# eth-cscs/COSTA

Hardware: AMD Instinct MI355X
Metric: GB/s device-resident tile pack+transpose+unpack (fp64), % HBM peak (higher is better)
Workload: dtype f64; 1 GPU; pxtran fp64 16384x16384, 256x256 blocks, op T, alpha=1 beta=0, 1x1 grid (BASELINE configs[1]); op=T, parallelism=1 rank(s), one per GPU, RCCL send/recv exchange, m=16384, n=16384, block=256, grid=1x1

## Files before the change

costa_amd/__init__.py:

```python
from __future__ import annotations

import ctypes as C
import os
import struct
from dataclasses import dataclass
from typing import Iterable, Sequence

import numpy as np

__all__ = [
    "CostaError", "lib", "FLOAT", "DOUBLE", "CFLOAT", "CDOUBLE", "INT32", "HALF", "BFLOAT16",
    "FP8_E4M3", "FP8_E5M2", "dtype_code", "element_code",
    "np_dtype", "Layout", "block_cyclic_layout", "custom_layout", "Comm", "transform",
    "transform_batch", "transform_async", "transform_batch_async", "synchronize", "transformer", "copy_and_transform", "execute_tiles", "execute_tiles_mixed",
    "convert_subtile", "TileOp", "TriOp", "TRI_OP_DTYPE", "transform_tri", "transform_tri_async",
    "execute_tiles_tri", "plan_export_tri", "tri_cut", "tri_subtile", "tri_phase_ms",
    "plan_export", "set_profiling", "get_stats", "release_caches", "TILE_OP_DTYPE",
    "ScaledOp", "SCALED_OP_DTYPE", "SCALED_F_ROWS", "transform_scaled", "execute_tiles_scaled",
    "plan_export_scaled", "scaled_subtile", "scaled_items",
    "transform_amax", "layout_amax", "execute_tiles_amax", "amax_items",
]

FLOAT, DOUBLE, CFLOAT, CDOUBLE, INT32 = 0, 1, 2, 3, 4
HALF, BFLOAT16 = 5, 6
# ... 179 lines not shown
        "costa_hip_transform_tri": (i, [vp, vp, c, c, i, vp, vp, vp]),
        "costa_hip_transform_tri_async": (i, [vp, vp, c, c, i, vp, vp, vp, vp]),
        "costa_hip_execute_tiles_tri": (i, [i, C.POINTER(TriOp), i64, vp, vp, vp, i, i]),
        "costa_hip_tri_cut": (i, []),
        "costa_hip_tri_phase_ms": (i, [C.POINTER(C.c_double), i]),
        "costa_hip_tri_subtile": (i, [i, C.POINTER(i), C.POINTER(i)]),
        "costa_hip_plan_export_tri": (i, [vp, vp, c, c, i, vp, vp, i, i, C.POINTER(TriPlanInfo), vp, vp,
                                          vp, vp, vp, vp, vp, vp, vp, vp]),
        "costa_hip_transform_scaled": (i, [vp, vp, c, vp, vp, vp, vp, vp]),
        "costa_hip_transform_scaled_async": (i, [vp, vp, c, vp, vp, vp, vp, vp, vp]),
        "costa_hip_execute_tiles_scaled": (i, [i, i, C.POINTER(ScaledOp), i64, vp, vp, vp, i, vp, vp, i]),
        "costa_hip_scaled_subtile": (i, [i, i, C.POINTER(i), C.POINTER(i)]),
        "costa_hip_scaled_items": (i, [C.POINTER(i64), i]),
        "costa_hip_transform_amax": (i, [vp, vp, c, vp, vp, vp, vp, vp, vp, vp]),
        "costa_hip_transform_amax_async": (i, [vp, vp, c, vp, vp, vp, vp, vp, vp, vp, vp]),
        "costa_hip_layout_amax": (i, [vp, vp, vp, vp]),
        "costa_hip_layout_amax_async": (i, [vp, vp, vp, vp, vp]),
        "costa_hip_execute_tiles_amax": (i, [i, i, C.POINTER(ScaledOp), i64, vp, vp, vp, i, vp, vp, vp, vp,
                                             i]),
        "costa_hip_amax_items": (i, [C.POINTER(i64), i]),
        "costa_hip_plan_export_scaled": (i, [vp, vp, c, vp, vp, i, i, C.POINTER(ScaledPlanInfo), vp, vp,
                                             vp, vp, vp, vp, vp, vp]),
        "costa_hip_plan_export": (i, [i, C.POINTER(vp), C.POINTER(vp), C.c_char_p, vp, vp, i, i,
                                      C.POINTER(PlanInfo), vp, vp, vp, vp, vp, vp, vp, vp]),
        "costa_hip_set_profiling": (i, [i]),
        "costa_hip_get_stats": (i, [C.POINTER(FullStats), i]),
        "costa_hip_release_caches": (i, []),
        "costa_hip_set_host_staging": (i, [i]),
        "costa_hip_set_planner": (i, [i]),
        "costa_hip_plan_export_device": (i, [i, i, C.POINTER(vp), C.POINTER(vp), C.c_char_p, vp, vp,
                                             i, i, C.POINTER(PlanInfo), vp, vp, vp, vp, vp, vp, vp,
                                             vp]),
        "costa_hip_set_list_builder": (i, [i]),
        "costa_hip_work_export": (i, [i, vp, i64, i, i, vp, i64, vp, i64, C.POINTER(i64)]),
    }
    for name, (res, args) in sig.items():
        try:
            f = getattr(L, name)
        except AttributeError:
            if os.environ.get("COSTA_LIB"):
                continue
            raise
        f.restype = res
        f.argtypes = args
    _lib = L
    return L


def _check(rc: int):
    if rc != 0:
        raise CostaError(rc, lib().costa_hip_last_error().decode(errors="replace"))


def _ptr(p) -> int:
    if p is None:
        return 0
    if isinstance(p, int):
        return p
    if isinstance(p, np.ndarray):
        return p.ctypes.data
    if hasattr(p, "data_ptr"):
        return p.data_ptr()
    raise TypeError(f"cannot take the address of {type(p)}")


def _scalar_bytes(code: int, x) -> bytes:
# ... 16 lines not shown
    row_start: int
    row_end: int
    col_start: int
    col_end: int
    data: int
    ld: int


class Layout:

    def __init__(self, handle: int, dtype: int, keep: Iterable = ()):
        self._h = C.c_void_p(handle)
        self.dtype = dtype
        self._keep = list(keep)

    @property
    def handle(self) -> C.c_void_p:
        return self._h

    def num_blocks(self) -> int:
        return lib().costa_hip_layout_num_blocks(self._h)

    def block(self, i: int) -> BlockInfo:
        v = [C.c_int() for _ in range(4)]
        d, ld = C.c_void_p(), C.c_int()
        _check(lib().costa_hip_layout_block(self._h, i, *[C.byref(x) for x in v], C.byref(d),
                                            C.byref(ld)))
        return BlockInfo(v[0].value, v[1].value, v[2].value, v[3].value, d.value or 0, ld.value)

    def shape(self) -> tuple:
        m, n = C.c_int(), C.c_int()
        _check(lib().costa_hip_layout_shape(self._h, C.byref(m), C.byref(n)))
        return m.value, n.value

    def reorder_ranks(self, reordering: Sequence[int]):
        p = np.ascontiguousarray(reordering, dtype=np.int32)
        _check(lib().costa_hip_layout_reorder_ranks(self._h, p.ctypes.data_as(C.POINTER(C.c_int)),
                                                    int(p.size)))

    def close(self):
        if self._h and self._h.value:
            lib().costa_hip_layout_destroy(self._h)
            self._h = C.c_void_p(0)

    def __del__(self):
        try:
            self.close()
        except Exception:
            pass


def block_cyclic_layout(m, n, block_m, block_n, i, j, sub_m, sub_n, p_m, p_n, order, rsrc, csrc,
                        ptr, lld, ordering, rank, dtype=DOUBLE) -> Layout:
    code = element_code(dtype)
    h = C.c_void_p()
    _check(lib().costa_hip_block_cyclic_layout(code, m, n, block_m, block_n, i, j, sub_m, sub_n,
                                               p_m, p_n, _chr(order), rsrc, csrc,
                                               C.c_void_p(_ptr(ptr)), lld, _chr(ordering), rank,
                                               C.byref(h)))
    return Layout(h.value, code, [ptr])


def custom_layout(rowblocks, colblocks, rowsplit, colsplit, owners, localblocks, ordering,
                  dtype=DOUBLE) -> Layout:
    code = element_code(dtype)
    rs = np.ascontiguousarray(rowsplit, dtype=np.int32)
# ... 459 lines not shown
    L = lib()
    args = (A.handle, Cl.handle, _chr(trans), ab, bb, rank, nranks, C.byref(info))
    _check(L.costa_hip_plan_export_scaled(*args, *([None] * 8)))
    b = info.base
    po = np.zeros(b.n_pack, TILE_OP_DTYPE)
    ls = np.zeros(info.n_local_scaled, SCALED_OP_DTYPE)
    us = np.zeros(info.n_unpack_scaled, SCALED_OP_DTYPE)
    cnt = [np.zeros(nranks, np.int64) for _ in range(4)]
    sc = np.zeros(2 * b.n_slots, _NP[code])
    _check(L.costa_hip_plan_export_scaled(*args, po.ctypes.data, ls.ctypes.data, us.ctypes.data,
                                          *[x.ctypes.data for x in cnt], sc.ctypes.data))
    return ScaledPlan(np.zeros(b.n_local, TILE_OP_DTYPE), po, np.zeros(b.n_unpack, TILE_OP_DTYPE), *cnt,
                      sc, b.send_elems, b.recv_elems, b.local_elems, ls, us)


def set_profiling(on: bool = True):
    _check(lib().costa_hip_set_profiling(int(on)))


def get_stats(reset: bool = False) -> dict:
    s = FullStats()
    _check(lib().costa_hip_get_stats(C.byref(s), int(reset)))
    return s.as_dict()


def release_caches():
    _check(lib().costa_hip_release_caches())


def set_planner(mode: int):
    _check(lib().costa_hip_set_planner(int(mode)))


def set_list_builder(mode: int):
    _check(lib().costa_hip_set_list_builder(int(mode)))


@dataclass
class WorkLists:
    ordered: np.ndarray
    work: np.ndarray
    meta: dict
    on_gpu: bool


_WORK_META = ("n_large", "n_medium", "n_skew", "n_cblock", "cblock_lds", "cb_map", "tiny_first",
              "n_tiny", "n_ordered", "n_work", "on_gpu", "flags")


def work_export(dtype, ops: np.ndarray, kind: str = "local", device=None) -> WorkLists:
    code = element_code(dtype)
    ops = np.ascontiguousarray(ops, dtype=TILE_OP_DTYPE)
    k = {"local": 0, "pack": 1, "unpack": 2}[kind]
    dev = -1 if device is None else int(device)
    meta = (C.c_int64 * 12)()
    L = lib()
    _check(L.costa_hip_work_export(code, ops.ctypes.data, ops.size, k, dev, None, 0, None, 0, meta))
    o = np.zeros(meta[8], TILE_OP_DTYPE)
    w = np.zeros(meta[9], np.uint64)
    _check(L.costa_hip_work_export(code, ops.ctypes.data, ops.size, k, dev, o.ctypes.data, o.size,
                                   w.ctypes.data, w.size, meta))
    m = dict(zip(_WORK_META, list(meta)))
    return WorkLists(o, w, m, bool(m["on_gpu"]))


def set_host_staging(mode: int):
# ... 8 lines not shown
```

costa_amd/csrc/capi.cpp:

```cpp
#include "engine.hpp"

#include <hip/hip_runtime.h>

#include <costa/transform.hpp>

#include <algorithm>
#include <cctype>
#include <complex>
#include <cstring>
#include <new>

struct costa_layout_s {
    costa::engine::elayout e;
    std::vector<int> base_owners;
};
struct costa_comm_s {
    costa::engine::comm* c = nullptr;
};

namespace {
thread_local std::string g_last_error;

template <typename F>
int guarded(F&& f) {
// ... 674 lines not shown
        [&](const std::vector<job>& jobs) { return costa::engine::make_plan(jobs, rank, nranks); },
        n, A, C, trans, alpha, beta, rank, nranks, info, local_ops, pack_ops, unpack_ops,
        send_counts, send_displs, recv_counts, recv_displs, scalars);
}

int costa_hip_plan_export_device(int device, int n, const costa_layout_t* A, const costa_layout_t* C,
                                 const char* trans, const void* alpha, const void* beta, int rank,
                                 int nranks, costa_plan_info_t* info, costa_tile_op_t* local_ops,
                                 costa_tile_op_t* pack_ops, costa_tile_op_t* unpack_ops,
                                 int64_t* send_counts, int64_t* send_displs, int64_t* recv_counts,
                                 int64_t* recv_displs, void* scalars) {
    device_restore keep;
    return export_plan(
        [&](const std::vector<job>& jobs) {
            auto p = costa::engine::make_plan_device(jobs, rank, nranks, 0, device, nullptr);
            if (!p)
                throw costa::engine::error(COSTA_ERR_ARG,
                                           "costa: the device planner does not apply to these "
                                           "layouts (local blocks are not exactly the rank's grid "
                                           "cells)");
            return p;
        },
        n, A, C, trans, alpha, beta, rank, nranks, info, local_ops, pack_ops, unpack_ops,
        send_counts, send_displs, recv_counts, recv_displs, scalars);
}

int costa_hip_set_planner(int mode) {
    return guarded([&] {
        if (mode < 0 || mode > 2) throw costa::engine::error(COSTA_ERR_ARG, "mode must be 0, 1 or 2");
        costa::engine::set_planner_mode(mode);
    });
}

int costa_hip_set_list_builder(int mode) {
    return guarded([&] {
        if (mode < 0 || mode > 2) throw costa::engine::error(COSTA_ERR_ARG, "mode must be 0, 1 or 2");
        costa::engine::set_list_builder_mode(mode);
    });
}

int costa_hip_work_export(int dtype, const costa_tile_op_t* ops, int64_t n_ops, int kind, int device,
                          costa_tile_op_t* ordered, int64_t cap_ordered, uint64_t* work,
                          int64_t cap_work, int64_t* meta) {
    auto body = [&] {
        if (!meta || (n_ops > 0 && !ops) || n_ops < 0) throw costa::engine::error(COSTA_ERR_ARG, "null argument");
        if (dtype < COSTA_FLOAT || dtype > COSTA_INT32) throw costa::engine::error(COSTA_ERR_ARG, "bad dtype");
        if (kind < 0 || kind > 2) throw costa::engine::error(COSTA_ERR_ARG, "kind must be 0, 1 or 2");
        std::vector<costa_tile_op_t> in(ops, ops + n_ops), o;
        std::vector<uint64_t> w;
        costa::engine::work_split ws;
        const bool on_gpu = costa::engine::work_export(
            costa_dtype_t(dtype), in, costa::engine::list_kind(kind), device, o, w, ws);
        const int64_t m[12] = {ws.n_large, ws.n_medium, ws.n_skew, ws.n_cblock, ws.cblock_lds, ws.cb_map,
                               ws.tiny_first, ws.n_tiny, int64_t(o.size()), int64_t(w.size()), on_gpu,
                               int64_t(ws.tr_shape) | int64_t(ws.sq) << 1 | int64_t(ws.full) << 2 |
                                   int64_t(ws.med_full) << 3 | int64_t(ws.med_sq) << 4 |
                                   int64_t(ws.skew_wide) << 5};
        std::memcpy(meta, m, sizeof(m));
        if (ordered && cap_ordered >= int64_t(o.size()) && !o.empty())
            std::memcpy(ordered, o.data(), o.size() * sizeof(o[0]));
        if (work && cap_work >= int64_t(w.size()) && !w.empty()) std::memcpy(work, w.data(), w.size() * sizeof(w[0]));
    };
    return device >= 0 ? gpu_guarded(body) : guarded(body);
}

int costa_hip_set_profiling(int on) {
// ... 166 lines not shown
```

costa_amd/csrc/engine.cpp:

```cpp
#include <exception>
#include <thread>
#include "engine.hpp"
#include "strip_work.hpp"

#include <hip/hip_runtime.h>
#include <rccl/rccl.h>

#include <algorithm>
#include <numeric>
#include <chrono>
#include <cmath>
#include <cstdio>
#include <cstdlib>
#include <cstring>
#include <deque>
#include <list>
#include <map>
#include <mutex>
#include <unordered_map>

namespace costa {
namespace engine {

#define HIP_CHECK(x)                                                                   \
// ... 1442 lines not shown
namespace {
int g_host_mode = -1;
}
int host_staging_mode() {
    if (g_host_mode < 0) {
        const char* s = std::getenv("COSTA_HOST_STAGING");
        g_host_mode = s ? (std::atoi(s) != 0) : 1;
    }
    return g_host_mode;
}
void set_host_staging_mode(int mode) {
    std::lock_guard<std::recursive_mutex> lk(g_mutex);
    g_host_mode = mode != 0;
}

namespace {

struct hasher {
    uint64_t h = 0x9E3779B97F4A7C15ull;
    uint64_t h2 = 0x2545F4914F6CDD1Dull;
    void mix(uint64_t v) {
        v ^= v >> 33;
        v *= 0xff51afd7ed558ccdull;
        v ^= v >> 33;
        h = (h ^ v) * 0xc4ceb9fe1a85ec53ull + 0x165667b19e3779f9ull;
        h ^= h >> 29;
        h2 = (h2 + v) * 0x9fb21c651e98df25ull;
        h2 ^= h2 >> 31;
    }
    void mix_vec(const std::vector<int>& v) {
        mix(v.size());
        for (int x : v) mix(uint64_t(uint32_t(x)));
    }
    void mix_layout(const elayout& L) {
        mix(uint64_t(L.dtype));
        mix(uint64_t(uint8_t(L.ordering)));
        mix(uint64_t(L.n_ranks));
        mix_vec(L.rows_split);
        mix_vec(L.cols_split);
        mix_vec(L.owners);
        mix(L.blocks.size());
        for (const auto& b : L.blocks) {
            mix(uint64_t(uint32_t(b.rows.start)) | (uint64_t(uint32_t(b.rows.end)) << 32));
            mix(uint64_t(uint32_t(b.cols.start)) | (uint64_t(uint32_t(b.cols.end)) << 32));
            mix(reinterpret_cast<uintptr_t>(b.data));
            mix(uint64_t(uint32_t(b.ld)));
        }
    }
};

}

uint64_t layout_hash(const elayout& L) {
    hasher h;
    h.mix_layout(L);
    return h.h | 1;
}

void layout_hashes(const elayout& L, uint64_t& h1, uint64_t& h2) {
    hasher h;
    h.mix_layout(L);
    h1 = h.h | 1;
    h2 = h.h2;
}

void set_layout_hash(elayout& L) { layout_hashes(L, L.hash, L.hash2); }

namespace {

struct cached_plan {
    std::unique_ptr<plan> p;
    int device = 0;
    bool staged = false;
    std::vector<hrange> h2d_ranges, d2h_ranges;
    dbuf stage;
    dbuf d_local, w_local, d_scal;
    work_split l_local;
    bool tr_local = true, ax_local = true;
    strip_list c_local;
    dbuf d_local_tri, w_local_tri;
    strip_list t_local;
    dbuf d_local_sc, w_local_sc;
    strip_list s_local;
    struct xround {
        dbuf d_pack, w_pack, d_unpack, w_unpack;
        work_split l_pack, l_unpack;
        strip_list c_pack, c_unpack;
        dbuf d_unpack_tri, w_unpack_tri;
        strip_list t_unpack;
        dbuf d_unpack_sc, w_unpack_sc;
        strip_list s_unpack;
        bool tr_unpack = false, ax_unpack = false;
    };
    std::vector<std::unique_ptr<xround>> rounds;
    std::vector<unsigned char> scal_host;
    std::shared_ptr<host_pipeline> pipe;
};

constexpr size_t kMaxPlans = 16;
struct keyed_plan {
    uint64_t h = 0;
    std::vector<uint64_t> key;
    std::unique_ptr<cached_plan> plan;
};
std::list<keyed_plan> g_plans;

void key_layout(std::vector<uint64_t>& k, const elayout& L) {
    uint64_t h1 = L.hash, h2 = L.hash2;
    if (!h1) layout_hashes(L, h1, h2);
    k.push_back(h1);
    k.push_back(h2);
    k.push_back(uint64_t(L.dtype) | uint64_t(uint8_t(L.ordering)) << 8 |
                uint64_t(uint32_t(L.n_ranks)) << 32);
    k.push_back(uint64_t(uint32_t(L.nbr())) | uint64_t(uint32_t(L.nbc())) << 32);
    k.push_back(L.blocks.size());
    if (!L.blocks.empty())
        for (const eblock* b : {&L.blocks.front(), &L.blocks.back()}) {
            k.push_back(reinterpret_cast<uintptr_t>(b->data));
            k.push_back(uint64_t(uint32_t(b->ld)) | uint64_t(uint32_t(b->rows.start)) << 32);
        }
}

elayout remap(const elayout& L, const std::vector<hrange>& ranges, char* dev) {
    elayout out = L;
    for (auto& b : out.blocks) {
        uintptr_t p = reinterpret_cast<uintptr_t>(b.data);
        auto it = std::upper_bound(ranges.begin(), ranges.end(), p,
                                   [](uintptr_t v, const hrange& r) { return v < r.lo; });
        if (it == ranges.begin()) throw error(COSTA_ERR_INTERNAL, "costa: staging map miss");
        --it;
        b.data = dev + it->dev_off + (p - it->lo);
    }
    return out;
}

std::vector<hrange> collect_ranges(const std::vector<const elayout*>& Ls) {
    std::vector<hrange> r;
    for (const elayout* L : Ls) {
        const size_t E = dtype_size(L->dtype);
        for (const auto& b : L->blocks) {
            size_t ext = block_extent_bytes(b, L->ordering, E);
            if (!ext) continue;
            uintptr_t lo = reinterpret_cast<uintptr_t>(b.data);
            r.push_back({lo, lo + ext, 0});
        }
    }
    std::sort(r.begin(), r.end(), [](const hrange& x, const hrange& y) { return x.lo < y.lo; });
    std::vector<hrange> m;
    for (const auto& x : r) {
        if (!m.empty() && x.lo <= m.back().hi)
            m.back().hi = std::max(m.back().hi, x.hi);
        else
            m.push_back(x);
    }
    return m;
}

// ... 4 lines not shown
constexpr size_t kDevicePlanBlocks = 4096;
constexpr size_t kColdDevicePlanBlocks = 100000;
bool g_device_planner_warm = false;
}

int planner_mode() {
    if (g_planner < 0) {
        const char* s = std::getenv("COSTA_PLANNER");
        g_planner = s ? std::max(0, std::min(2, std::atoi(s))) : 1;
    }
    return g_planner;
}

void set_planner_mode(int mode) {
    std::lock_guard<std::recursive_mutex> lk(g_mutex);
    g_planner = mode;
}

namespace {
int g_list_builder = -1;
}

int list_builder_mode() {
    if (g_list_builder < 0) {
        const char* s = std::getenv("COSTA_LIST_BUILDER");
        g_list_builder = s ? std::max(0, std::min(2, std::atoi(s))) : 1;
    }
    return g_list_builder;
}

void set_list_builder_mode(int mode) {
    std::lock_guard<std::recursive_mutex> lk(g_mutex);
    g_list_builder = mode;
}

namespace {
template <typename X>
void upload_list(dbuf& d, const std::vector<X>& h, const X* sec, size_t at, size_t n, hipStream_t s) {
    if (!sec || n == 0) return d.upload(h, s);
    const size_t total = h.size() + n;
    d.reserve(total * sizeof(X));
    X* p = static_cast<X*>(d.p);
    if (at) HIP_CHECK(hipMemcpyAsync(p, h.data(), at * sizeof(X), hipMemcpyHostToDevice, s));
    HIP_CHECK(hipMemcpyAsync(p + at, sec, n * sizeof(X), hipMemcpyDeviceToDevice, s));
    if (h.size() > at)
        HIP_CHECK(hipMemcpyAsync(p + at + n, h.data() + at, (h.size() - at) * sizeof(X), hipMemcpyHostToDevice, s));
}
}

bool work_export(costa_dtype_t dtype, const std::vector<costa_tile_op_t>& ops, list_kind kind, int device,
                 std::vector<costa_tile_op_t>& ordered, std::vector<uint64_t>& work, work_split& w) {
    std::lock_guard<std::recursive_mutex> lk(g_mutex);
    if (device < 0) {
        w = build_work(dtype, ops, ordered, work, kind);
        return false;
    }
    device_ctx& dc = ctx(device);
    device_section sec;
    sec.device = device;
    sec.stream = dc.main;
    sec.force = true;
    w = build_work(dtype, ops, ordered, work, kind, &sec);
    if (!sec.n_ordered) return false;
    std::vector<costa_tile_op_t> o(sec.n_ordered);
    std::vector<uint64_t> k(sec.n_work);
    HIP_CHECK(hipMemcpyAsync(o.data(), sec.d_ordered, o.size() * sizeof(o[0]), hipMemcpyDeviceToHost, dc.main));
    HIP_CHECK(hipMemcpyAsync(k.data(), sec.d_work, k.size() * sizeof(k[0]), hipMemcpyDeviceToHost, dc.main));
    HIP_CHECK(hipStreamSynchronize(dc.main));
    ordered.insert(ordered.begin() + std::ptrdiff_t(sec.at_ordered), o.begin(), o.end());
    work.insert(work.begin() + std::ptrdiff_t(sec.at_work), k.begin(), k.end());
    return true;
}

namespace {
std::unique_ptr<plan> plan_jobs(const std::vector<job>& jobs, comm* c, hipStream_t s) {
    const int lb = c->size == 1 && c->nccl ? loopback_exchange() : 0;
    const int mode = planner_mode();
    size_t blocks = 0;
    for (const job& j : jobs) blocks += j.A->blocks.size() + j.C->blocks.size();
    const size_t need = g_device_planner_warm ? kDevicePlanBlocks : kColdDevicePlanBlocks;
    if (mode == 2 || (mode == 1 && blocks >= need)) {
        if (auto p = make_plan_device(jobs, c->rank, c->size, lb, c->device, s)) {
            g_stats.device_plans++;
            g_device_planner_warm = true;
            return p;
        }
    }
    return make_plan(jobs, c->rank, c->size, lb);
}

cached_plan* get_plan(const std::vector<job>& jobs, comm* c, device_ctx& dc) {
    std::vector<uint64_t> key;
    key.reserve(4 + jobs.size() * 30);
    key.push_back(uint64_t(uint32_t(c->rank)) | uint64_t(uint32_t(c->size)) << 32);
    key.push_back(uint64_t(uint32_t(c->device)) | uint64_t(uint32_t(host_staging_mode())) << 32);
    key.push_back(jobs.size());
    for (const auto& j : jobs) {
        key_layout(key, *j.A);
        key_layout(key, *j.C);
        uint64_t w = uint64_t(uint8_t(std::toupper(static_cast<unsigned char>(j.trans))));
        for (bool cm : {true, false})
            w = w << 8 | scale_kind(j.C->dtype, j.s, cm, std::toupper(j.trans) == 'C');
        key.push_back(w);
        key.push_back(uint64_t(uint8_t(std::toupper(static_cast<unsigned char>(j.uplo)))) << 32 |
                      uint64_t(j.scaled) << 40 | uint64_t(uint32_t(j.k)));
    }
    hasher h;
    for (uint64_t w : key) h.mix(w);
    for (auto it = g_plans.begin(); it != g_plans.end(); ++it) {
        if (it->h == h.h && it->key == key) {
            g_plans.splice(g_plans.begin(), g_plans, it);
            g_stats.plan_hits++;
            return g_plans.front().plan.get();
        }
    }
    g_stats.plan_misses++;
    static const bool trace = std::getenv("COSTA_PLAN_TRACE") != nullptr;
    auto now = [] {
        return std::chrono::duration<double, std::milli>(
                   std::chrono::steady_clock::now().time_since_epoch()).count();
    };
    const double t0 = now();
    double t_resid = 0, t_plan = 0, t_work = 0;

    const bool half = any_half(jobs);
    const bool fp8 = any_fp8(jobs);
    const bool mixed = any_mixed(jobs) || half || fp8;
    const bool masked = any_masked(jobs);
    const bool scaled = any_scaled(jobs);
    if (mixed || masked || scaled) {
        costa_dtype_t a, b;
        check_jobs(jobs, c->size, a, b);
    }
    auto cp = std::make_unique<cached_plan>();
    cp->device = c->device;
    bool all_dev = true;
    std::vector<const elayout*> host_layouts;
    std::vector<bool> on_dev;
    for (const auto& j : jobs)
        for (const elayout* L : {j.A, j.C}) {
            bool d = layout_on_device(*L);
            on_dev.push_back(d);
            all_dev = all_dev && d;
        }
    std::vector<elayout> remapped;
    std::vector<job> pj = jobs;
    std::vector<hrange> staged_ranges;
    std::vector<uint8_t> range_flags;
    if (!all_dev && mixed)
        throw error(COSTA_ERR_ARG,
                    fp8  ? "costa: FP8 transforms (A or C of a 1-byte element type) need "
                           "device-resident layouts"
                    : half ? "costa: half-precision transforms (A or C of a 2-byte element type) need "
                           "device-resident layouts"
                         : "costa: mixed-precision transforms (A and C of different element types) need "
                           "device-resident layouts");
    if (!all_dev && scaled)
        throw error(COSTA_ERR_ARG, "costa: scaled transforms need device-resident layouts");
    if (!all_dev) {
        cp->staged = true;
        std::vector<const elayout*> As, Cs;
        size_t k = 0;
        for (const auto& j : jobs) {
            if (!on_dev[k++]) As.push_back(j.A);
            if (!on_dev[k++]) Cs.push_back(j.C);
        }
        std::vector<const elayout*> all = As;
        all.insert(all.end(), Cs.begin(), Cs.end());
// ... 37 lines not shown
        if (pipe_ok) {
            const double tp = now();
            auto hplan = plan_jobs(jobs, c, dc.main);
            g_stats.plan_ms += now() - tp;
            if (host_pipeline_accepts(hplan->dtype, hplan->pack_ops)) {
                cp->staged = false;
                cp->p = std::move(hplan);
                const int R = c->exchanges() ? exchange_rounds() : 1;
                std::vector<int> pr, ur;
                exchange_round_of_ops(*cp->p, R, pr, ur);
                cp->pipe = make_host_pipeline(cp->p->dtype, cp->p->pack_ops, cp->p->local_ops,
                                              cp->p->unpack_ops, pr, ur, R);
                g_plans.push_front({h.h, std::move(key), std::move(cp)});
                while (g_plans.size() > kMaxPlans) g_plans.pop_back();
                return g_plans.front().plan.get();
            }
        }
        cp->stage.reserve(std::max<size_t>(off, 256));
        staged_ranges = ranges;
        remapped.reserve(jobs.size() * 2);
        k = 0;
        for (auto& j : pj) {
            if (!on_dev[k++]) {
                remapped.push_back(remap(*j.A, ranges, static_cast<char*>(cp->stage.p)));
                j.A = &remapped.back();
            }
            if (!on_dev[k++]) {
                remapped.push_back(remap(*j.C, ranges, static_cast<char*>(cp->stage.p)));
                j.C = &remapped.back();
            }
        }
    }
    t_resid = now() - t0;
    cp->p = plan_jobs(pj, c, dc.main);
    const plan& p = *cp->p;
    t_plan = now() - t0 - t_resid;
    g_stats.plan_ms += t_plan;
    if (cp->staged) {
        const size_t E = dtype_size(p.dtype);
        const uintptr_t base = reinterpret_cast<uintptr_t>(cp->stage.p);
        std::vector<size_t> written(staged_ranges.size(), 0);
        std::vector<bool> reads_c(staged_ranges.size(), false);
        auto account = [&](const std::vector<costa_tile_op_t>& ops) {
            for (const auto& op : ops) {
                if (op.dst < base) continue;
                const size_t off = size_t(op.dst - base);
                auto it = std::upper_bound(staged_ranges.begin(), staged_ranges.end(), off,
                                           [](size_t v, const hrange& r) { return v < r.dev_off; });
                if (it == staged_ranges.begin()) continue;
                const size_t i = size_t(it - staged_ranges.begin()) - 1;
                if (off >= staged_ranges[i].dev_off + (staged_ranges[i].hi - staged_ranges[i].lo))
                    continue;
                written[i] += size_t(op.nf) * size_t(op.ns) * E;
                if (((op.flags & COSTA_SCALE_MASK) >> COSTA_SCALE_SHIFT) == COSTA_SCALE_AXPBY)
                    reads_c[i] = true;
            }
        };
        account(p.local_ops);
        account(p.unpack_ops);
        for (size_t i = 0; i < staged_ranges.size(); ++i) {
            const hrange& r = staged_ranges[i];
            const uint8_t f = range_flags[i];
            const bool overwritten = !masked && f == 2 && !reads_c[i] && written[i] == r.hi - r.lo;
            if ((f & 1) || ((f & 2) && !overwritten)) cp->h2d_ranges.push_back(r);
            if (f & 2) cp->d2h_ranges.push_back(r);
        }
// ... 230 lines not shown

namespace {
void issue_exchange(comm* c, const plan& p, char* sb, char* rb, hipStream_t s, int round = 0,
                    int rounds = 1) {
    const size_t E = dtype_size(p.pkg_dtype);
    const size_t piece = max_message_bytes();
    NCCL_CHECK(ncclGroupStart());
    for (int q = 0; q < c->size; ++q) {
        int64_t slo, shi, rlo, rhi;
        round_range(p.send_counts[size_t(q)], E, rounds, round, slo, shi);
        round_range(p.recv_counts[size_t(q)], E, rounds, round, rlo, rhi);
        const size_t sbytes = size_t(shi - slo) * E, rbytes = size_t(rhi - rlo) * E;
        char* sp = sb + size_t(p.send_displs[size_t(q)] + slo) * E;
        char* rp = rb + size_t(p.recv_displs[size_t(q)] + rlo) * E;
        for (size_t o = 0; o < sbytes; o += piece)
            NCCL_CHECK(ncclSend(sp + o, std::min(piece, sbytes - o), ncclUint8, q, c->nccl, s));
        for (size_t o = 0; o < rbytes; o += piece)
            NCCL_CHECK(ncclRecv(rp + o, std::min(piece, rbytes - o), ncclUint8, q, c->nccl, s));
    }
    NCCL_CHECK(ncclGroupEnd());
}

struct scaled_args {
    const void *row_scale = nullptr, *col_scale = nullptr;
    void *row_amax = nullptr, *col_amax = nullptr;
    bool amax() const { return row_amax || col_amax; }
};

void launch_local(const cached_plan& cp, const scaled_args& sv, phase_timer& tm, hipStream_t ls) {
    const plan& p = *cp.p;
    if (cp.c_local.n_items) {
        tm.start(PH_LOCAL, ls);
        launch_convert(p.src_dtype, p.dtype, static_cast<const costa_tile_op_t*>(cp.d_local.p),
                       static_cast<const uint64_t*>(cp.w_local.p), cp.c_local, nullptr, nullptr,
                       cp.d_scal.p, ls);
        tm.stop();
    }
    if (cp.l_local.n_items()) {
        tm.start(PH_LOCAL, ls);
        launch_tiles(p.dtype,
                     make_launch(cp.l_local, cp.d_local.p, cp.w_local.p, nullptr, nullptr,
                                 cp.d_scal.p, cp.tr_local, cp.ax_local),
                     ls);
        tm.stop();
    }
    if (cp.t_local.n_items) {
        tm.start(PH_TRI_LOCAL, ls);
        launch_tri(p.dtype, static_cast<const costa_tri_op_t*>(cp.d_local_tri.p),
                   static_cast<const uint64_t*>(cp.w_local_tri.p), cp.t_local, nullptr, nullptr,
                   cp.d_scal.p, ls);
        tm.stop();
    }

    if (cp.s_local.n_items) {
        tm.start(PH_LOCAL, ls);
        launch_scaled(p.src_dtype, p.dtype, static_cast<const costa_scaled_op_t*>(cp.d_local_sc.p),
                      static_cast<const uint64_t*>(cp.w_local_sc.p), cp.s_local, nullptr, nullptr,
                      cp.d_scal.p, sv.row_scale, sv.col_scale, sv.row_amax, sv.col_amax, ls);
        tm.stop();
    }
}

void launch_pack_round(const cached_plan& cp, const cached_plan::xround& x, char* sb, phase_timer& tm,
                       hipStream_t s) {
    const plan& p = *cp.p;
    if (x.c_pack.n_items) {
        tm.start(PH_PACK, s);
        launch_convert(p.src_dtype, p.pkg_dtype, static_cast<const costa_tile_op_t*>(x.d_pack.p),
                       static_cast<const uint64_t*>(x.w_pack.p), x.c_pack, nullptr, sb,
                       cp.d_scal.p, s);
        tm.stop();
    }
    if (x.l_pack.n_items()) {
        tm.start(PH_PACK, s);
        launch_tiles(p.pkg_dtype,
                     make_launch(x.l_pack, x.d_pack.p, x.w_pack.p, nullptr, sb, cp.d_scal.p,
                                 false, false),
                     s);
        tm.stop();
    }
}

void launch_unpack_round(const cached_plan& cp, const cached_plan::xround& x, const char* rb,
                         const scaled_args& sv, phase_timer& tm, hipStream_t s, hipEvent_t moved) {
    const plan& p = *cp.p;
    if (x.c_unpack.n_items) {
        if (moved) HIP_CHECK(hipStreamWaitEvent(s, moved, 0));
        tm.start(PH_UNPACK, s);
        launch_convert(p.pkg_dtype, p.dtype, static_cast<const costa_tile_op_t*>(x.d_unpack.p),
                       static_cast<const uint64_t*>(x.w_unpack.p), x.c_unpack, rb, nullptr,
                       cp.d_scal.p, s);
        tm.stop();
    }
    if (x.l_unpack.n_items()) {
        if (moved) HIP_CHECK(hipStreamWaitEvent(s, moved, 0));
        tm.start(PH_UNPACK, s);
        launch_tiles(p.dtype,
                     make_launch(x.l_unpack, x.d_unpack.p, x.w_unpack.p, rb, nullptr,
                                 cp.d_scal.p, x.tr_unpack, x.ax_unpack),
                     s);
        tm.stop();
    }
    if (x.t_unpack.n_items) {
        if (moved) HIP_CHECK(hipStreamWaitEvent(s, moved, 0));
        tm.start(PH_TRI_UNPACK, s);
        launch_tri(p.dtype, static_cast<const costa_tri_op_t*>(x.d_unpack_tri.p),
                   static_cast<const uint64_t*>(x.w_unpack_tri.p), x.t_unpack, rb, nullptr,
                   cp.d_scal.p, s);
        tm.stop();
    }
    if (x.s_unpack.n_items) {
        if (moved) HIP_CHECK(hipStreamWaitEvent(s, moved, 0));
        tm.start(PH_UNPACK, s);
        launch_scaled(p.pkg_dtype, p.dtype, static_cast<const costa_scaled_op_t*>(x.d_unpack_sc.p),
                      static_cast<const uint64_t*>(x.w_unpack_sc.p), x.s_unpack, rb, nullptr,
                      cp.d_scal.p, sv.row_scale, sv.col_scale, sv.row_amax, sv.col_amax, s);
        tm.stop();
    }
}

void count_items(const plan& p, const work_split& w) {
    g_stats.tile_items += w.n_large + w.n_medium;
    g_stats.skew_items += w.n_skew;
    g_stats.cblock_items += w.n_cblock;
    g_stats.tiny_items += w.n_tiny;
    if (!dtype_is_complex(p.dtype) && pieces_in_group_launch(w.n_cblock, w.n_tiny))
        g_stats.fused_pieces += w.n_tiny;
}

void count_local(const cached_plan& cp, bool amax) {
    const plan& p = *cp.p;
    g_stats.tri_items += cp.t_local.n_items;
    g_scaled_items += cp.s_local.n_items;
    if (amax) g_amax_items += cp.s_local.n_items;
    if (cp.l_local.n_items() || cp.c_local.n_items || cp.t_local.n_items || cp.s_local.n_items) {
        g_stats.local_launches++;
        g_stats.local_bytes += p.local_bytes;
        count_items(p, cp.l_local);
        g_stats.convert_items += cp.c_local.n_items;
    }
}

void count_pack_round(const cached_plan& cp, const cached_plan::xround& x) {
    g_stats.pack_launches += x.l_pack.n_items() || x.c_pack.n_items ? 1 : 0;
    count_items(*cp.p, x.l_pack);
    g_stats.convert_items += x.c_pack.n_items;
}

// ... 476 lines not shown
```

costa_amd/csrc/engine.hpp:

```cpp
#pragma once

#include <costa/layout.hpp>
#include <costa_hip.h>

#include <array>
#include <cstdint>
#include <functional>
#include <memory>
#include <string>
#include <vector>

namespace costa {
namespace engine {

size_t dtype_size(costa_dtype_t t);
bool dtype_is_complex(costa_dtype_t t);
bool dtype_is_half(costa_dtype_t t);
costa_dtype_t compute_dtype(costa_dtype_t src, costa_dtype_t dst);
bool half_pair(costa_dtype_t src, costa_dtype_t dst);
bool dtype_is_fp8(costa_dtype_t t);
bool fp8_pair(costa_dtype_t src, costa_dtype_t dst);
costa_dtype_t plan_pkg_dtype(costa_dtype_t src, costa_dtype_t dst);

struct eblock {
    interval rows, cols;
    char* data = nullptr;
    int ld = 0;
};

struct elayout {
    costa_dtype_t dtype = COSTA_DOUBLE;
    std::vector<int> rows_split, cols_split;
    std::vector<int> owners;
    int n_ranks = 1;
    char ordering = 'C';
    std::vector<eblock> blocks;
    uint64_t hash = 0;
    uint64_t hash2 = 0;

    int nbr() const { return int(rows_split.size()) - 1; }
    int nbc() const { return int(cols_split.size()) - 1; }
};

template <typename T>
costa_dtype_t dtype_of();

template <typename T>
elayout erase(const grid_layout<T>& L);

uint64_t layout_hash(const elayout& L);
void layout_hashes(const elayout& L, uint64_t& h1, uint64_t& h2);
void set_layout_hash(elayout& L);

struct scal {
    std::array<unsigned char, 16> alpha{};
    std::array<unsigned char, 16> beta{};
};

struct job {
    const elayout* A = nullptr;
    const elayout* C = nullptr;
    char trans = 'N';
    scal s;
    char uplo = 'A';
    int k = 0;
    bool scaled = false;
    const void* row_scale = nullptr;
    const void* col_scale = nullptr;
    void* row_amax = nullptr;
    void* col_amax = nullptr;
};

struct plan {
    costa_dtype_t dtype = COSTA_DOUBLE;
    costa_dtype_t src_dtype = COSTA_DOUBLE;
    costa_dtype_t pkg_dtype = COSTA_DOUBLE;
    bool mixed() const { return src_dtype != dtype; }
    bool half() const { return dtype_is_half(src_dtype) || dtype_is_half(dtype); }
    bool fp8() const { return dtype_is_fp8(src_dtype) || dtype_is_fp8(dtype); }
    bool converting() const { return mixed() || half() || fp8(); }
    costa_dtype_t scalar_dtype() const { return compute_dtype(src_dtype, dtype); }
    int rank = 0, n_ranks = 1;
    std::vector<costa_tile_op_t> local_ops, pack_ops, unpack_ops;
    std::vector<costa_tri_op_t> local_tri, unpack_tri;
    bool scaled = false;
// ... 268 lines not shown
```

include/costa_hip.h:

```cpp
#ifndef COSTA_HIP_H
#define COSTA_HIP_H

#include <stddef.h>
#include <stdint.h>

#ifdef __cplusplus
extern "C" {
#endif

#define COSTA_OK 0
#define COSTA_ERR_ARG 1
#define COSTA_ERR_HIP 2
#define COSTA_ERR_NCCL 3
#define COSTA_ERR_INTERNAL 4

typedef enum {
    COSTA_FLOAT = 0,
    COSTA_DOUBLE = 1,
    COSTA_CFLOAT = 2,
    COSTA_CDOUBLE = 3,
    COSTA_INT32 = 4,
    COSTA_HALF = 5,
    COSTA_BFLOAT16 = 6,
    COSTA_FP8_E4M3 = 7,
// ... 195 lines not shown

typedef struct {
    double pack_ms, local_ms, unpack_ms, exchange_ms, h2d_ms, d2h_ms;
    int64_t pack_launches, local_launches, unpack_launches;
    int64_t pack_bytes, local_bytes, unpack_bytes;
    int64_t transforms;
    int64_t plan_hits, plan_misses;
    int64_t host_groups;
    int64_t device_plans;
    double plan_ms;
    int64_t host_direct;
    int64_t host_direct_groups;
    int64_t tile_items, skew_items, cblock_items, tiny_items;
    int64_t device_lists;
    int64_t fused_pieces;
    int64_t convert_items;
    int64_t tri_items;
} costa_stats_t;
int costa_hip_tri_phase_ms(double* ms, int reset);
int costa_hip_set_profiling(int on);
int costa_hip_get_stats(costa_stats_t* out, int reset);
int costa_hip_release_caches(void);

int costa_hip_set_host_staging(int mode);

int costa_hip_set_planner(int mode);
int costa_hip_plan_export_device(int device, int n, const costa_layout_t* A, const costa_layout_t* C,
                                 const char* trans, const void* alpha, const void* beta, int rank,
                                 int nranks, costa_plan_info_t* info, costa_tile_op_t* local_ops,
                                 costa_tile_op_t* pack_ops, costa_tile_op_t* unpack_ops,
                                 int64_t* send_counts, int64_t* send_displs, int64_t* recv_counts,
                                 int64_t* recv_displs, void* scalars);

int costa_hip_set_list_builder(int mode);
int costa_hip_work_export(int dtype, const costa_tile_op_t* ops, int64_t n_ops, int kind, int device,
                          costa_tile_op_t* ordered, int64_t cap_ordered, uint64_t* work,
                          int64_t cap_work, int64_t* meta);

#ifdef __cplusplus
}
#endif
#endif
```

Before: 6467 GB/s.

## Make cached plans relocatable across buffer addresses via anchor-relative layout hashing

```diff
diff --git a/costa_amd/__init__.py b/costa_amd/__init__.py
--- a/costa_amd/__init__.py
+++ b/costa_amd/__init__.py
@@ -235,6 +235,8 @@
                                              i, i, C.POINTER(PlanInfo), vp, vp, vp, vp, vp, vp, vp,
                                              vp]),
         "costa_hip_set_list_builder": (i, [i]),
+        "costa_hip_set_plan_relocation": (i, [i]),
+        "costa_hip_layout_structure": (i, [vp, C.POINTER(C.c_uint64), C.POINTER(i64)]),
         "costa_hip_work_export": (i, [i, vp, i64, i, i, vp, i64, vp, i64, C.POINTER(i64)]),
     }
     for name, (res, args) in sig.items():
@@ -317,6 +319,11 @@
         m, n = C.c_int(), C.c_int()
         _check(lib().costa_hip_layout_shape(self._h, C.byref(m), C.byref(n)))
         return m.value, n.value
+
+    def structure(self) -> tuple:
+        h, s = (C.c_uint64 * 2)(), (C.c_int64 * 2)()
+        _check(lib().costa_hip_layout_structure(self._h, h, s))
+        return h[0], h[1], s[0], s[1]
 
     def reorder_ranks(self, reordering: Sequence[int]):
         p = np.ascontiguousarray(reordering, dtype=np.int32)
@@ -842,6 +849,10 @@
     _check(lib().costa_hip_set_planner(int(mode)))
 
 
+def set_plan_relocation(on: bool = True):
+    _check(lib().costa_hip_set_plan_relocation(int(on)))
+
+
 def set_list_builder(mode: int):
     _check(lib().costa_hip_set_list_builder(int(mode)))
 
diff --git a/costa_amd/csrc/capi.cpp b/costa_amd/csrc/capi.cpp
--- a/costa_amd/csrc/capi.cpp
+++ b/costa_amd/csrc/capi.cpp
@@ -730,6 +730,21 @@
     });
 }
 
+int costa_hip_set_plan_relocation(int on) {
+    return guarded([&] { costa::engine::set_plan_relocation(on != 0); });
+}
+
+int costa_hip_layout_structure(costa_layout_t layout, uint64_t* hashes, int64_t* span) {
+    return guarded([&] {
+        if (!layout || !hashes || !span) throw costa::engine::error(COSTA_ERR_ARG, "null argument");
+        const costa::engine::layout_structure s = costa::engine::structure_of(layout->e);
+        hashes[0] = s.h1;
+        hashes[1] = s.h2;
+        span[0] = s.lo;
+        span[1] = s.hi;
+    });
+}
+
 int costa_hip_set_list_builder(int mode) {
     return guarded([&] {
         if (mode < 0 || mode > 2) throw costa::engine::error(COSTA_ERR_ARG, "mode must be 0, 1 or 2");
diff --git a/costa_amd/csrc/engine.cpp b/costa_amd/csrc/engine.cpp
--- a/costa_amd/csrc/engine.cpp
+++ b/costa_amd/csrc/engine.cpp
@@ -1498,7 +1498,7 @@
         mix(v.size());
         for (int x : v) mix(uint64_t(uint32_t(x)));
     }
-    void mix_layout(const elayout& L) {
+    void mix_layout(const elayout& L, uintptr_t anchor) {
         mix(uint64_t(L.dtype));
         mix(uint64_t(uint8_t(L.ordering)));
         mix(uint64_t(L.n_ranks));
@@ -1506,10 +1506,11 @@
         mix_vec(L.cols_split);
         mix_vec(L.owners);
         mix(L.blocks.size());
+        mix(uint64_t(anchor % 256));
         for (const auto& b : L.blocks) {
             mix(uint64_t(uint32_t(b.rows.start)) | (uint64_t(uint32_t(b.rows.end)) << 32));
             mix(uint64_t(uint32_t(b.cols.start)) | (uint64_t(uint32_t(b.cols.end)) << 32));
-            mix(reinterpret_cast<uintptr_t>(b.data));
+            mix(uint64_t(reinterpret_cast<uintptr_t>(b.data) - anchor));
             mix(uint64_t(uint32_t(b.ld)));
         }
     }
@@ -1517,20 +1518,36 @@
 
 }
 
-uint64_t layout_hash(const elayout& L) {
+layout_structure structure_of(const elayout& L) {
+    if (L.shash) return {L.shash, L.shash2, L.anchor, L.span_lo, L.span_hi};
+    layout_structure s;
+    if (!L.blocks.empty()) s.anchor = reinterpret_cast<uintptr_t>(L.blocks.front().data);
     hasher h;
-    h.mix_layout(L);
-    return h.h | 1;
-}
-
-void layout_hashes(const elayout& L, uint64_t& h1, uint64_t& h2) {
-    hasher h;
-    h.mix_layout(L);
-    h1 = h.h | 1;
-    h2 = h.h2;
-}
-
-void set_layout_hash(elayout& L) { layout_hashes(L, L.hash, L.hash2); }
+    h.mix_layout(L, s.anchor);
+    s.h1 = h.h | 1;
+    s.h2 = h.h2;
+    const size_t E = dtype_size(L.dtype);
+    bool any = false;
+    for (const auto& b : L.blocks) {
+        const int64_t ext = int64_t(block_extent_bytes(b, L.ordering, E));
+        if (!ext) continue;
+        const int64_t o = int64_t(reinterpret_cast<uintptr_t>(b.data) - s.anchor);
+        s.lo = any ? std::min(s.lo, o) : o;
+        s.hi = any ? std::max(s.hi, o + ext) : o + ext;
+        any = true;
+    }
+    return s;
+}
+
+void set_layout_hash(elayout& L) {
+    L.shash = 0;
+    const layout_structure s = structure_of(L);
+    L.shash = s.h1;
+    L.shash2 = s.h2;
+    L.anchor = s.anchor;
+    L.span_lo = s.lo;
+    L.span_hi = s.hi;
+}
 
 namespace {
 
@@ -1561,6 +1578,12 @@
     std::vector<std::unique_ptr<xround>> rounds;
     std::vector<unsigned char> scal_host;
     std::shared_ptr<host_pipeline> pipe;
+    std::vector<uintptr_t> anchors;
+    std::vector<char> overlap;
+    bool relocatable = false;
+    int64_t da = 0, dc = 0;
+    const char* a_base() const { return reinterpret_cast<const char*>(uintptr_t(da)); }
+    char* c_base() const { return reinterpret_cast<char*>(uintptr_t(dc)); }
 };
 
 constexpr size_t kMaxPlans = 16;
@@ -1571,24 +1594,60 @@
 };
 std::list<keyed_plan> g_plans;
 
-void key_layout(std::vector<uint64_t>& k, const elayout& L) {
-    uint64_t h1 = L.hash, h2 = L.hash2;
-    if (!h1) layout_hashes(L, h1, h2);
-    k.push_back(h1);
-    k.push_back(h2);
-    k.push_back(uint64_t(L.dtype) | uint64_t(uint8_t(L.ordering)) << 8 |
+void key_layout(std::vector<uint64_t>& k, const elayout& L, const layout_structure& s) {
+    k.push_back(s.h1);
+    k.push_back(s.h2);
+    k.push_back(uint64_t(L.dtype) | uint64_t(uint8_t(L.ordering)) << 8 | uint64_t(s.anchor % 256) << 16 |
                 uint64_t(uint32_t(L.n_ranks)) << 32);
     k.push_back(uint64_t(uint32_t(L.nbr())) | uint64_t(uint32_t(L.nbc())) << 32);
     k.push_back(L.blocks.size());
     if (!L.blocks.empty())
         for (const eblock* b : {&L.blocks.front(), &L.blocks.back()}) {
-            k.push_back(reinterpret_cast<uintptr_t>(b->data));
+            k.push_back(uint64_t(reinterpret_cast<uintptr_t>(b->data) - s.anchor));
             k.push_back(uint64_t(uint32_t(b->ld)) | uint64_t(uint32_t(b->rows.start)) << 32);
         }
+}
+
+bool spans_overlap(const layout_structure& a, const layout_structure& c) {
+    if (a.lo >= a.hi || c.lo >= c.hi) return false;
+    return a.anchor + uintptr_t(a.lo) < c.anchor + uintptr_t(c.hi) &&
+           c.anchor + uintptr_t(c.lo) < a.anchor + uintptr_t(a.hi);
+}
+
+bool replay_at(cached_plan& cp, const std::vector<layout_structure>& st) {
+    if (st.size() != cp.anchors.size()) return false;
+    bool same = true;
+    for (size_t i = 0; i < st.size() && same; ++i) same = st[i].anchor == cp.anchors[i];
+    cp.da = cp.dc = 0;
+    if (same) return true;
+    if (!cp.relocatable || !plan_relocation()) return false;
+    int64_t d[2] = {0, 0};
+    bool have[2] = {false, false};
+    for (size_t i = 0; i < st.size(); ++i) {
+        if (st[i].lo >= st[i].hi) continue;
+        const int64_t di = int64_t(st[i].anchor - cp.anchors[i]);
+        if (have[i & 1] && d[i & 1] != di) return false;
+        d[i & 1] = di;
+        have[i & 1] = true;
+    }
+    if (d[0] % 256 != 0 || d[1] % 256 != 0) return false;
+    for (size_t t = 0; 2 * t < st.size(); ++t) {
+        const bool o = spans_overlap(st[2 * t], st[2 * t + 1]);
+        if (o != bool(cp.overlap[t]) || (o && d[0] != d[1])) return false;
+    }
+    for (size_t i = 0; i < st.size(); ++i) {
+        if (st[i].lo >= st[i].hi || d[i & 1] == 0) continue;
+        const char* at = reinterpret_cast<const char*>(st[i].anchor);
+        if (!is_device_ptr(at + st[i].lo) || !is_device_ptr(at + st[i].hi - 1)) return false;
+    }
+    cp.da = d[0];
+    cp.dc = d[1];
+    return true;
 }
 
 elayout remap(const elayout& L, const std::vector<hrange>& ranges, char* dev) {
     elayout out = L;
+    out.shash = 0;
     for (auto& b : out.blocks) {
         uintptr_t p = reinterpret_cast<uintptr_t>(b.data);
         auto it = std::upper_bound(ranges.begin(), ranges.end(), p,
@@ -1659,6 +1718,23 @@
 void set_list_builder_mode(int mode) {
     std::lock_guard<std::recursive_mutex> lk(g_mutex);
     g_list_builder = mode;
+}
+
+namespace {
+int g_relocate = -1;
+}
+
+bool plan_relocation() {
+    if (g_relocate < 0) {
+        const char* s = std::getenv("COSTA_PLAN_RELOCATE");
+        g_relocate = s ? (std::atoi(s) != 0) : 1;
+    }
+    return g_relocate != 0;
+}
+
+void set_plan_relocation(bool on) {
+    std::lock_guard<std::recursive_mutex> lk(g_mutex);
+    g_relocate = on;
 }
 
 namespace {
@@ -1722,9 +1798,13 @@
     key.push_back(uint64_t(uint32_t(c->rank)) | uint64_t(uint32_t(c->size)) << 32);
     key.push_back(uint64_t(uint32_t(c->device)) | uint64_t(uint32_t(host_staging_mode())) << 32);
     key.push_back(jobs.size());
+    std::vector<layout_structure> st;
+    st.reserve(2 * jobs.size());
     for (const auto& j : jobs) {
-        key_layout(key, *j.A);
-        key_layout(key, *j.C);
+        for (const elayout* L : {j.A, j.C}) {
+            st.push_back(structure_of(*L));
+            key_layout(key, *L, st.back());
+        }
         uint64_t w = uint64_t(uint8_t(std::toupper(static_cast<unsigned char>(j.trans))));
         for (bool cm : {true, false})
             w = w << 8 | scale_kind(j.C->dtype, j.s, cm, std::toupper(j.trans) == 'C');
@@ -1735,7 +1815,7 @@
     hasher h;
     for (uint64_t w : key) h.mix(w);
     for (auto it = g_plans.begin(); it != g_plans.end(); ++it) {
-        if (it->h == h.h && it->key == key) {
+        if (it->h == h.h && it->key == key && replay_at(*it->plan, st)) {
             g_plans.splice(g_plans.begin(), g_plans, it);
             g_stats.plan_hits++;
             return g_plans.front().plan.get();
@@ -1761,6 +1841,10 @@
     }
     auto cp = std::make_unique<cached_plan>();
     cp->device = c->device;
+    for (size_t i = 0; i < st.size(); ++i) {
+        cp->anchors.push_back(st[i].anchor);
+        if (i & 1) cp->overlap.push_back(spans_overlap(st[i - 1], st[i]));
+    }
     bool all_dev = true;
     std::vector<const elayout*> host_layouts;
     std::vector<bool> on_dev;
@@ -1864,6 +1948,7 @@
         }
     }
     t_resid = now() - t0;
+    cp->relocatable = all_dev;
     cp->p = plan_jobs(pj, c, dc.main);
     const plan& p = *cp->p;
     t_plan = now() - t0 - t_resid;
@@ -2160,14 +2245,14 @@
     if (cp.c_local.n_items) {
         tm.start(PH_LOCAL, ls);
         launch_convert(p.src_dtype, p.dtype, static_cast<const costa_tile_op_t*>(cp.d_local.p),
-                       static_cast<const uint64_t*>(cp.w_local.p), cp.c_local, nullptr, nullptr,
+                       static_cast<const uint64_t*>(cp.w_local.p), cp.c_local, cp.a_base(), cp.c_base(),
                        cp.d_scal.p, ls);
         tm.stop();
     }
     if (cp.l_local.n_items()) {
         tm.start(PH_LOCAL, ls);
         launch_tiles(p.dtype,
-                     make_launch(cp.l_local, cp.d_local.p, cp.w_local.p, nullptr, nullptr,
+                     make_launch(cp.l_local, cp.d_local.p, cp.w_local.p, cp.a_base(), cp.c_base(),
                                  cp.d_scal.p, cp.tr_local, cp.ax_local),
                      ls);
         tm.stop();
@@ -2175,7 +2260,7 @@
     if (cp.t_local.n_items) {
         tm.start(PH_TRI_LOCAL, ls);
         launch_tri(p.dtype, static_cast<const costa_tri_op_t*>(cp.d_local_tri.p),
-                   static_cast<const uint64_t*>(cp.w_local_tri.p), cp.t_local, nullptr, nullptr,
+                   static_cast<const uint64_t*>(cp.w_local_tri.p), cp.t_local, cp.a_base(), cp.c_base(),
                    cp.d_scal.p, ls);
         tm.stop();
     }
@@ -2183,7 +2268,7 @@
     if (cp.s_local.n_items) {
         tm.start(PH_LOCAL, ls);
         launch_scaled(p.src_dtype, p.dtype, static_cast<const costa_scaled_op_t*>(cp.d_local_sc.p),
-                      static_cast<const uint64_t*>(cp.w_local_sc.p), cp.s_local, nullptr, nullptr,
+                      static_cast<const uint64_t*>(cp.w_local_sc.p), cp.s_local, cp.a_base(), cp.c_base(),
                       cp.d_scal.p, sv.row_scale, sv.col_scale, sv.row_amax, sv.col_amax, ls);
         tm.stop();
     }
@@ -2195,14 +2280,14 @@
     if (x.c_pack.n_items) {
         tm.start(PH_PACK, s);
         launch_convert(p.src_dtype, p.pkg_dtype, static_cast<const costa_tile_op_t*>(x.d_pack.p),
-                       static_cast<const uint64_t*>(x.w_pack.p), x.c_pack, nullptr, sb,
+                       static_cast<const uint64_t*>(x.w_pack.p), x.c_pack, cp.a_base(), sb,
                        cp.d_scal.p, s);
         tm.stop();
     }
     if (x.l_pack.n_items()) {
         tm.start(PH_PACK, s);
         launch_tiles(p.pkg_dtype,
-                     make_launch(x.l_pack, x.d_pack.p, x.w_pack.p, nullptr, sb, cp.d_scal.p,
+                     make_launch(x.l_pack, x.d_pack.p, x.w_pack.p, cp.a_base(), sb, cp.d_scal.p,
                                  false, false),
                      s);
         tm.stop();
@@ -2216,7 +2301,7 @@
         if (moved) HIP_CHECK(hipStreamWaitEvent(s, moved, 0));
         tm.start(PH_UNPACK, s);
         launch_convert(p.pkg_dtype, p.dtype, static_cast<const costa_tile_op_t*>(x.d_unpack.p),
-                       static_cast<const uint64_t*>(x.w_unpack.p), x.c_unpack, rb, nullptr,
+                       static_cast<const uint64_t*>(x.w_unpack.p), x.c_unpack, rb, cp.c_base(),
                        cp.d_scal.p, s);
         tm.stop();
     }
@@ -2224,7 +2309,7 @@
         if (moved) HIP_CHECK(hipStreamWaitEvent(s, moved, 0));
         tm.start(PH_UNPACK, s);
         launch_tiles(p.dtype,
-                     make_launch(x.l_unpack, x.d_unpack.p, x.w_unpack.p, rb, nullptr,
+                     make_launch(x.l_unpack, x.d_unpack.p, x.w_unpack.p, rb, cp.c_base(),
                                  cp.d_scal.p, x.tr_unpack, x.ax_unpack),
                      s);
         tm.stop();
@@ -2233,7 +2318,7 @@
         if (moved) HIP_CHECK(hipStreamWaitEvent(s, moved, 0));
         tm.start(PH_TRI_UNPACK, s);
         launch_tri(p.dtype, static_cast<const costa_tri_op_t*>(x.d_unpack_tri.p),
-                   static_cast<const uint64_t*>(x.w_unpack_tri.p), x.t_unpack, rb, nullptr,
+                   static_cast<const uint64_t*>(x.w_unpack_tri.p), x.t_unpack, rb, cp.c_base(),
                    cp.d_scal.p, s);
         tm.stop();
     }
@@ -2241,7 +2326,7 @@
         if (moved) HIP_CHECK(hipStreamWaitEvent(s, moved, 0));
         tm.start(PH_UNPACK, s);
         launch_scaled(p.pkg_dtype, p.dtype, static_cast<const costa_scaled_op_t*>(x.d_unpack_sc.p),
-                      static_cast<const uint64_t*>(x.w_unpack_sc.p), x.s_unpack, rb, nullptr,
+                      static_cast<const uint64_t*>(x.w_unpack_sc.p), x.s_unpack, rb, cp.c_base(),
                       cp.d_scal.p, sv.row_scale, sv.col_scale, sv.row_amax, sv.col_amax, s);
         tm.stop();
     }
diff --git a/costa_amd/csrc/engine.hpp b/costa_amd/csrc/engine.hpp
--- a/costa_amd/csrc/engine.hpp
+++ b/costa_amd/csrc/engine.hpp
@@ -35,8 +35,9 @@
     int n_ranks = 1;
     char ordering = 'C';
     std::vector<eblock> blocks;
-    uint64_t hash = 0;
-    uint64_t hash2 = 0;
+    uint64_t shash = 0, shash2 = 0;
+    uintptr_t anchor = 0;
+    int64_t span_lo = 0, span_hi = 0;
 
     int nbr() const { return int(rows_split.size()) - 1; }
     int nbc() const { return int(cols_split.size()) - 1; }
@@ -48,9 +49,15 @@
 template <typename T>
 elayout erase(const grid_layout<T>& L);
 
-uint64_t layout_hash(const elayout& L);
-void layout_hashes(const elayout& L, uint64_t& h1, uint64_t& h2);
+struct layout_structure {
+    uint64_t h1 = 0, h2 = 0;
+    uintptr_t anchor = 0;
+    int64_t lo = 0, hi = 0;
+};
+layout_structure structure_of(const elayout& L);
 void set_layout_hash(elayout& L);
+bool plan_relocation();
+void set_plan_relocation(bool on);
 
 struct scal {
     std::array<unsigned char, 16> alpha{};
diff --git a/include/costa_hip.h b/include/costa_hip.h
--- a/include/costa_hip.h
+++ b/include/costa_hip.h
@@ -251,6 +251,9 @@
                                  int64_t* send_counts, int64_t* send_displs, int64_t* recv_counts,
                                  int64_t* recv_displs, void* scalars);
 
+int costa_hip_set_plan_relocation(int on);
+int costa_hip_layout_structure(costa_layout_t layout, uint64_t* hashes, int64_t* span);
+
 int costa_hip_set_list_builder(int mode);
 int costa_hip_work_export(int dtype, const costa_tile_op_t* ops, int64_t n_ops, int kind, int device,
                           costa_tile_op_t* ordered, int64_t cap_ordered, uint64_t* work,
```

New measurement: 6467 GB/s. No clear change (-0.0%).
